# Hiroshiba/realtime-yukarin

Measured on NVIDIA H100. Metric: chunks_per_s_0.3s_24kHz_encode_stage1_stage2_vocode, higher is better.
Workload: dtype f64 (WORLD analysis / synthesis, SPTK), f16 operands / f32 accumulate: stage-2 k4 layers on wgmma, stage-1 k4 layers on mma.sync inside the one-launch cluster kernel; f32 CUDA cores (3x3 / k3 edge layers)

## Files before the change

### realtime_yukarin_b200/csrc/conv.h

```cpp
#pragma once
#include <cuda.h>

#include "common.cuh"

namespace ryk {

enum Act { ACT_NONE = 0, ACT_LEAKY = 1, ACT_RELU = 2 };
enum DType { DT_F32 = 0, DT_F16 = 1 };

constexpr int kMaxGroupVoices = 8;
constexpr int kMaxGroupBatch = 64;

struct LayerWeights {
  const float* w[kMaxGroupVoices];
  const float* scale[kMaxGroupVoices];
  const float* shift[kMaxGroupVoices];
  float host_scale[kMaxGroupVoices], host_shift[kMaxGroupVoices];
  uint8_t voice_of[kMaxGroupBatch];
};
__host__ __device__ inline int item_voice(const LayerWeights& wt, int b) { return b < kMaxGroupBatch ? wt.voice_of[b] : 0; }
struct TcWeightMaps { CUtensorMap m[kMaxGroupVoices]; };

struct ConvLayer {
  int transposed = 0;
  int B = 1, Hin = 1, Win = 1, Hout = 1, Wout = 1;
  int C0 = 0, C1 = 0, Cout = 0;
  int KH = 1, KW = 1, SH = 1, SW = 1, PH = 0, PW = 0;
  int act = ACT_NONE;
  int band_y0 = 0, band_y1 = 0;
  int skip_y0 = 0, skip_y1 = 0;
  int run_y0 = 0, run_y1 = 0;
  const void* in0 = nullptr; const void* in1 = nullptr; int in_dtype = DT_F32;
  void* out = nullptr; int out_dtype = DT_F32;
  int n_voices = 1;
  LayerWeights wt = {};
  bool host_scale_valid = false;
  const __half* w_tc[kMaxGroupVoices] = {};
  const __half* w_frag = nullptr;
  int ksplit = 1;
  int ksplit_tiles = 0;
  CUtensorMap tmA0, tmA1, tmO;
  TcWeightMaps tmB;
  int tile_w = 0, tile_h = 0;
  int block_n = 0;
  bool tc_ready = false;
};

inline int layer_class_rows(const ConvLayer& L) { return L.transposed ? L.Hin : L.Hout; }
inline int layer_band_end(const ConvLayer& L) { return L.band_y1 > 0 ? L.band_y1 : layer_class_rows(L); }
inline void layer_band_out_rows(const ConvLayer& L, int* r0, int* r1) {
  const int s = L.transposed ? L.SH : 1;
  *r0 = L.band_y0 * s;
  *r1 = layer_band_end(L) * s < L.Hout ? layer_band_end(L) * s : L.Hout;
}

int pack_weights_direct(const float* d_w_chainer, int transposed, int Cin, int Cout, int KH, int KW, float* d_out, cudaStream_t st);
int pack_weights_tc(const float* d_w_chainer, int transposed, int Cin, int Cout, int KH, int KW, int SH, int SW, __half* d_out, cudaStream_t st);

int conv_direct_run(const ConvLayer& L, cudaStream_t st);
bool conv_direct_band_supported(const ConvLayer& L);
bool conv_direct_cin1(const ConvLayer& L);
constexpr int kCin1Rows = 8;
bool conv_direct_per_item_weights(const ConvLayer& L);

bool tc_layer_eligible(const ConvLayer& L);
int tc_init();
int tc_layer_prepare(ConvLayer& L, int num_sms);
int tc_layer_weight_maps(ConvLayer& L);
int conv_tc_run(const ConvLayer& L, cudaStream_t st);
int tc_tile_rows(const ConvLayer& L);
int tc_tile_count(const ConvLayer& L);

int s1_pack_weights(const float* d_w_chainer, int transposed, int Cin, int Cout, __half* d_out, cudaStream_t st);
int s1_fused_init();
int s1_fused_cluster_size();

}
```

### realtime_yukarin_b200/csrc/conv_tc.cu

```cuda
#include <cuda.h>
#include <cudaTypedefs.h>

#include "conv.h"
#include "tc_ptx.cuh"

namespace ryk {

struct TcParams {
  int transposed, B, Hout, Wout, Cout;
  int Hc, Wc;
  int tile_w, tile_h, tiles_w, tiles_h;
  int th0;
  int skip_t0, skip_tn;
  int run_y0, run_y1;
  int chunks0, chunks1;
  int taps_w, ntaps;
  int sh, sw, ph, pw;
  int classes_w;
  int ksplit, chunks_per_split;
  int act;
  LayerWeights wt;
  __half* out;
};

template <int BLOCK_N>
__device__ __forceinline__ void wgmma_tile(float (&acc)[BLOCK_N / 2], uint64_t adesc, uint64_t bdesc) {
  if constexpr (BLOCK_N == 128) wgmma_m64n128(acc, adesc, bdesc);
  else wgmma_m64n64(acc, adesc, bdesc);
}

constexpr int kMaxSplits = 16;

__device__ __forceinline__ void add4(float4& a, const float4& b) { a.x += b.x; a.y += b.y; a.z += b.z; a.w += b.w; }

__device__ __forceinline__ float4 splitk_sum(const float4 (&v)[kMaxSplits], int ks) {
  float4 a = v[0];
  if (ks <= 4) {
#pragma unroll
    for (int s = 1; s < 4; ++s) if (s < ks) add4(a, v[s]);
    return a;
  }
#pragma unroll
  for (int g = 0; g < 8; ++g) {
    float4 part = make_float4(0.f, 0.f, 0.f, 0.f);
    if (g < ks) add4(part, v[g]);
    if (g + 8 < ks) add4(part, v[g + 8]);
    if (g == 0) a = part; else add4(a, part);
  }
  return a;
}

template <int BLOCK_N>
__device__ __forceinline__ uint32_t partial_offset(int row, int c) { return (uint32_t)(row * BLOCK_N * 4 + ((c ^ (row & 7)) << 4)); }

template <int BLOCK_N, int kStages, int kMinBlocks>
__global__ void __launch_bounds__(kTcThreads, kMinBlocks)
k_conv_tc(const __grid_constant__ CUtensorMap tmA0, const __grid_constant__ CUtensorMap tmA1,
          const __grid_constant__ TcWeightMaps tmB, const __grid_constant__ CUtensorMap tmO, const __grid_constant__ TcParams p) {
  static_assert(BLOCK_N == 64 || BLOCK_N == 128, "BLOCK_N");
  extern __shared__ __align__(1024) uint8_t smem_raw[];
  constexpr uint32_t kABytes = kBlockM * kBlockK * 2;
  constexpr uint32_t kBBytes = BLOCK_N * kBlockK * 2;
  static_assert((size_t)kBlockM * BLOCK_N * 4 <= (size_t)kStages * (kABytes + kBBytes), "epilogue staging must fit the stage buffers");
  uint8_t* smem = (uint8_t*)(((uintptr_t)smem_raw + 1023) & ~(uintptr_t)1023);
  uint8_t* smem_a = smem;
  uint8_t* smem_b = smem + kStages * kABytes;
  uint64_t* full_bar = (uint64_t*)(smem_b + kStages * kBBytes);
  uint64_t* empty_bar = full_bar + kStages;
  float* s_scale = (float*)(((uintptr_t)(empty_bar + kStages) + 15) & ~(uintptr_t)15);
  float* s_shift = s_scale + BLOCK_N;

  const int warp = threadIdx.x >> 5;
  pdl_trigger();

  int mt = blockIdx.x;
  const int tw = mt % p.tiles_w; mt /= p.tiles_w;
  int th = mt % p.tiles_h + p.th0; mt /= p.tiles_h;
  th += th >= p.skip_t0 ? p.skip_tn : 0;
  const int b = mt;
  const int n0 = blockIdx.y * BLOCK_N;
  const int cls = blockIdx.z / p.ksplit, split = blockIdx.z % p.ksplit;
  const int py = cls / p.classes_w, px = cls % p.classes_w;
  const int oy0 = th * p.tile_h, ox0 = tw * p.tile_w;
  const int chunks_per_tap = p.chunks0 + p.chunks1;
  const int total_chunks = p.ntaps * chunks_per_tap;
  const int kc_begin = split * p.chunks_per_split;
  const int kc_end = min(total_chunks, kc_begin + p.chunks_per_split);
  const int my_chunks = kc_end - kc_begin;
  const int voice = item_voice(p.wt, b);
  const CUtensorMap* tmBv = &tmB.m[voice];

  if (threadIdx.x == kTcConsumers) {
    asm volatile("prefetch.tensormap [%0];" ::"l"(&tmA0) : "memory");
    asm volatile("prefetch.tensormap [%0];" ::"l"(tmBv) : "memory");
    if (p.chunks1 > 0) asm volatile("prefetch.tensormap [%0];" ::"l"(&tmA1) : "memory");
    if (p.ksplit == 1) asm volatile("prefetch.tensormap [%0];" ::"l"(&tmO) : "memory");
    for (int i = 0; i < kStages; ++i) { mbar_init(&full_bar[i], 1); mbar_init(&empty_bar[i], kTcConsumers / 32); }
    asm volatile("fence.mbarrier_init.release.cluster;" ::: "memory");
  }
  if (threadIdx.x < kTcConsumers) {
    const float* scale = p.wt.scale[voice]; const float* shift = p.wt.shift[voice];
    for (int i = threadIdx.x; i < BLOCK_N; i += kTcConsumers) { s_scale[i] = __ldg(scale + n0 + i); s_shift[i] = __ldg(shift + n0 + i); }
  }
  __syncthreads();
  pdl_wait();

  if (warp == kTcConsumers / 32) {
    for (int i = 0; i < my_chunks; ++i) {
      const int s = i % kStages;
      const uint32_t ph = (i / kStages) & 1;
      mbar_wait(&empty_bar[s], ph ^ 1);
      const int kc = kc_begin + i;
      const int tap = kc / chunks_per_tap;
      const int cc = kc - tap * chunks_per_tap;
      const int ty = tap / p.taps_w, tx = tap - ty * p.taps_w;
      int ix, iy;
      if (!p.transposed) {
        ix = ox0 * p.sw + tx - p.pw; iy = oy0 * p.sh + ty - p.ph;
        if (iy >= p.run_y0 && iy + p.sh * (p.tile_h - 1) < p.run_y1) iy = p.run_y0;
      }
      else {
        ix = p.sw == 2 ? ox0 + tx - 1 + px : ox0;
        iy = p.sh == 2 ? oy0 + ty - 1 + py : oy0;
      }
      if (elect_one()) {
        mbar_expect_tx(&full_bar[s], kABytes + kBBytes);
        if (cc < p.chunks0) tma_load_4d(smem_a + s * kABytes, &tmA0, &full_bar[s], cc * kBlockK, ix, iy, b);
        else tma_load_4d(smem_a + s * kABytes, &tmA1, &full_bar[s], (cc - p.chunks0) * kBlockK, ix, iy, b);
        tma_load_2d(smem_b + s * kBBytes, tmBv, &full_bar[s], kc * kBlockK, cls * p.Cout + n0);
      }
    }
    if (p.ksplit > 1) { cluster_sync_all(); cluster_sync_all(); }
  } else if (warp < kTcConsumers / 32) {
    const int g = threadIdx.x >> 7, wl = warp & 3, lane = threadIdx.x & 31;
    float acc[BLOCK_N / 2];
#pragma unroll
    for (int i = 0; i < BLOCK_N / 2; ++i) acc[i] = 0.f;
    wgmma_fence_acc(acc);
    for (int i = 0; i < my_chunks; ++i) {
      const int s = i % kStages;
      mbar_wait(&full_bar[s], (i / kStages) & 1);
      const uint64_t adesc = make_sw128_desc(smem_u32(smem_a + s * kABytes + g * (64 * 128)));
      const uint64_t bdesc = make_sw128_desc(smem_u32(smem_b + s * kBBytes));
      wgmma_fence();
#pragma unroll
      for (int k = 0; k < kBlockK / kMmaK; ++k) wgmma_tile<BLOCK_N>(acc, adesc + (uint64_t)(k * 2), bdesc + (uint64_t)(k * 2));
      wgmma_commit();
      wgmma_wait<1>();
      wgmma_fence_acc(acc);
      if (i > 0) {
        __syncwarp();
        if (lane == 0) mbar_arrive(&empty_bar[(i - 1) % kStages]);
      }
    }
    wgmma_wait<0>();
    wgmma_fence_acc(acc);
    asm volatile("bar.sync 1, %0;" ::"n"(kTcConsumers) : "memory");
    const int rbase = g * 64 + wl * 16 + (lane >> 2);
    const int cq = 2 * (lane & 3);
    if (p.ksplit > 1) {
#pragma unroll
      for (int i = 0; i < BLOCK_N / 2; i += 2) {
        const int row = rbase + 8 * ((i >> 1) & 1);
        const int col = 8 * (i >> 2) + cq;
        *reinterpret_cast<float2*>(smem + partial_offset<BLOCK_N>(row, col >> 2) + (col & 3) * 4) = make_float2(acc[i], acc[i + 1]);
      }
      cluster_sync_all();
      const int vw = min(p.tile_w, p.Wc - ox0), vh = min(p.tile_h, p.Hc - oy0);
      constexpr int kChunks = BLOCK_N / 4;
      const int total = vw * vh * kChunks;
      const int j1 = (int)((long long)total * (split + 1) / p.ksplit);
      const uint32_t partial = smem_u32(smem);
      for (int j = (int)((long long)total * split / p.ksplit) + threadIdx.x; j < j1; j += kTcConsumers) {
        const int q = j / kChunks, c = j - q * kChunks;
        const int y = q / vw, x = q - y * vw;
        const uint32_t off = partial + partial_offset<BLOCK_N>(y * p.tile_w + x, c);
        float4 v[kMaxSplits];
#pragma unroll
        for (int s = 0; s < kMaxSplits; ++s)
          if (s < p.ksplit) v[s] = ld_cluster_f4(cluster_map(off, s));
        const float4 a = splitk_sum(v, p.ksplit);
        const int n = 4 * c;
        float o[4] = {fmaf(a.x, s_scale[n], s_shift[n]), fmaf(a.y, s_scale[n + 1], s_shift[n + 1]),
                      fmaf(a.z, s_scale[n + 2], s_shift[n + 2]), fmaf(a.w, s_scale[n + 3], s_shift[n + 3])};
#pragma unroll
        for (int k = 0; k < 4; ++k) {
          if (p.act == ACT_LEAKY) o[k] = o[k] > 0.f ? o[k] : 0.2f * o[k]; else if (p.act == ACT_RELU) o[k] = fmaxf(o[k], 0.f);
        }
        const int ys = p.transposed ? (oy0 + y) * p.sh + py : oy0 + y;
        const int xs = p.transposed ? (ox0 + x) * p.sw + px : ox0 + x;
        __half2 h0 = __floats2half2_rn(o[0], o[1]), h1 = __floats2half2_rn(o[2], o[3]);
        *reinterpret_cast<uint2*>(p.out + (((size_t)b * p.Hout + ys) * p.Wout + xs) * p.Cout + n0 + n) =
            make_uint2(*reinterpret_cast<uint32_t*>(&h0), *reinterpret_cast<uint32_t*>(&h1));
      }
      cluster_sync_all();
      return;
    }
#pragma unroll
    for (int i = 0; i < BLOCK_N / 2; i += 2) {
      const int row = rbase + 8 * ((i >> 1) & 1);
      const int col = 8 * (i >> 2) + cq;
      float v0 = fmaf(acc[i], s_scale[col], s_shift[col]);
      float v1 = fmaf(acc[i + 1], s_scale[col + 1], s_shift[col + 1]);
      if (p.act == ACT_LEAKY) { v0 = v0 > 0.f ? v0 : 0.2f * v0; v1 = v1 > 0.f ? v1 : 0.2f * v1; }
      else if (p.act == ACT_RELU) { v0 = fmaxf(v0, 0.f); v1 = fmaxf(v1, 0.f); }
      uint8_t* blk = smem + (col >> 6) * (kBlockM * 128) + row * 128;
      *reinterpret_cast<__half2*>(blk + ((((col & 63) >> 3) ^ (row & 7)) << 4) + (col & 7) * 2) = __floats2half2_rn(v0, v1);
    }
    if (my_chunks > 0) {
      asm volatile("fence.proxy.async.shared::cta;" ::: "memory");
      asm volatile("bar.sync 1, %0;" ::"n"(kTcConsumers) : "memory");
      if (threadIdx.x == 0) {
        const int xs = p.transposed ? ox0 * p.sw + px : ox0;
        const int ys = p.transposed ? oy0 * p.sh + py : oy0;
#pragma unroll
        for (int jb = 0; jb < BLOCK_N / 64; ++jb)
          asm volatile("cp.async.bulk.tensor.4d.global.shared::cta.bulk_group [%0, {%2, %3, %4, %5}], [%1];"
                       ::"l"(&tmO), "r"(smem_u32(smem + jb * (kBlockM * 128))), "r"(n0 + jb * 64), "r"(xs), "r"(ys), "r"(b) : "memory");
        asm volatile("cp.async.bulk.commit_group;" ::: "memory");
        asm volatile("cp.async.bulk.wait_group.read 0;" ::: "memory");
      }
    }
  }
}

static PFN_cuTensorMapEncodeTiled_v12000 g_encode = nullptr;
static int g_clusters[kMaxSplits + 1] = {};

template <int BN, int ST> static constexpr size_t tc_smem_bytes() {
  return (size_t)ST * (kBlockM * kBlockK * 2 + BN * kBlockK * 2) + 2 * ST * 8 + 16 + 1024 + 2 * BN * 4 + 32;
}
#define RYK_TC_N128 k_conv_tc<128, 3, 2>
#define RYK_TC_N64 k_conv_tc<64, 4, 2>

int tc_init() {
  if (!g_encode) {
    void* fn = nullptr;
    cudaDriverEntryPointQueryResult qres;
    RYK_CUDA(cudaGetDriverEntryPoint("cuTensorMapEncodeTiled", &fn, cudaEnableDefault, &qres));
    RYK_CHECK(qres == cudaDriverEntryPointSuccess && fn != nullptr, "cuTensorMapEncodeTiled not available from the driver");
    g_encode = (PFN_cuTensorMapEncodeTiled_v12000)fn;
  }
  RYK_CUDA(cudaFuncSetAttribute(RYK_TC_N128, cudaFuncAttributeMaxDynamicSharedMemorySize, (int)tc_smem_bytes<128, 3>()));
  RYK_CUDA(cudaFuncSetAttribute(RYK_TC_N64, cudaFuncAttributeMaxDynamicSharedMemorySize, (int)tc_smem_bytes<64, 4>()));
  RYK_CUDA(cudaFuncSetAttribute(RYK_TC_N128, cudaFuncAttributeNonPortableClusterSizeAllowed, 1));
  RYK_CUDA(cudaFuncSetAttribute(RYK_TC_N64, cudaFuncAttributeNonPortableClusterSizeAllowed, 1));
  if (g_clusters[1] == 0) {
    auto active = [](auto kernel, size_t smem, int ks) {
      cudaLaunchConfig_t cfg = {};
      cfg.gridDim = dim3(1, 1, ks); cfg.blockDim = dim3(kTcThreads); cfg.dynamicSmemBytes = smem;
      cudaLaunchAttribute at[1];
      at[0].id = cudaLaunchAttributeClusterDimension; at[0].val.clusterDim.x = 1; at[0].val.clusterDim.y = 1; at[0].val.clusterDim.z = ks;
      cfg.attrs = at; cfg.numAttrs = 1;
      int n = 0;
      if (cudaOccupancyMaxActiveClusters(&n, kernel, &cfg) != cudaSuccess) { cudaGetLastError(); n = 0; }
      return n;
    };
    for (int ks = 1; ks <= kMaxSplits; ++ks)
      g_clusters[ks] = std::min(active(RYK_TC_N128, tc_smem_bytes<128, 3>(), ks), active(RYK_TC_N64, tc_smem_bytes<64, 4>(), ks));
    RYK_CHECK(g_clusters[1] > 0, "the tensor-core convolution kernel does not fit an SM");
  }
  return 0;
}


bool tc_layer_eligible(const ConvLayer& L) {
  const bool k2d = L.KH == 4 && L.KW == 4 && L.SH == 2 && L.SW == 2 && L.PH == 1 && L.PW == 1;
  const bool k1d = L.KH == 1 && L.KW == 4 && L.SH == 1 && L.SW == 2 && L.PH == 0 && L.PW == 1;
  if (!k2d && !k1d) return false;
  if (L.C0 % kBlockK != 0 || L.C1 % kBlockK != 0 || L.C0 == 0) return false;
  if (L.Cout % 64 != 0) return false;
  if (L.in_dtype != DT_F16 || L.out_dtype != DT_F16) return false;
  return true;
}

static int pow2_floor(int v) { int p = 1; while (p * 2 <= v) p *= 2; return p; }

static int make_act_map(CUtensorMap* m, const void* ptr, int C, int W, int H, int B, int box_w, int box_h, int stride_w, int stride_h) {
  cuuint64_t dims[4] = {(cuuint64_t)C, (cuuint64_t)W, (cuuint64_t)H, (cuuint64_t)B};
  cuuint64_t strides[3] = {(cuuint64_t)C * 2, (cuuint64_t)W * C * 2, (cuuint64_t)H * W * C * 2};
  cuuint32_t box[4] = {(cuuint32_t)kBlockK, (cuuint32_t)(box_w * stride_w), (cuuint32_t)(box_h * stride_h), 1};
  cuuint32_t estr[4] = {1, (cuuint32_t)stride_w, (cuuint32_t)stride_h, 1};
  CUresult r = g_encode(m, CU_TENSOR_MAP_DATA_TYPE_FLOAT16, 4, const_cast<void*>(ptr), dims, strides, box, estr,
                        CU_TENSOR_MAP_INTERLEAVE_NONE, CU_TENSOR_MAP_SWIZZLE_128B, CU_TENSOR_MAP_L2_PROMOTION_L2_256B,
                        CU_TENSOR_MAP_FLOAT_OOB_FILL_NONE);
  if (r != CUDA_SUCCESS) { set_error("cuTensorMapEncodeTiled(activation) failed: " + std::to_string((int)r)); return -1; }
  return 0;
}

static int make_weight_map(CUtensorMap* m, const void* ptr, size_t K, size_t rows, int block_n) {
  cuuint64_t dims[2] = {(cuuint64_t)K, (cuuint64_t)rows};
  cuuint64_t strides[1] = {(cuuint64_t)K * 2};
  cuuint32_t box[2] = {(cuuint32_t)kBlockK, (cuuint32_t)block_n};
  cuuint32_t estr[2] = {1, 1};
  CUresult r = g_encode(m, CU_TENSOR_MAP_DATA_TYPE_FLOAT16, 2, const_cast<void*>(ptr), dims, strides, box, estr,
                        CU_TENSOR_MAP_INTERLEAVE_NONE, CU_TENSOR_MAP_SWIZZLE_128B, CU_TENSOR_MAP_L2_PROMOTION_L2_256B,
                        CU_TENSOR_MAP_FLOAT_OOB_FILL_NONE);
  if (r != CUDA_SUCCESS) { set_error("cuTensorMapEncodeTiled(weights) failed: " + std::to_string((int)r)); return -1; }
  return 0;
}

static void tc_tile_shape(const ConvLayer& L, int* tile_w, int* tile_h) {
  const int Wc = L.transposed ? L.Win : L.Wout;
  *tile_w = pow2_floor(Wc < kBlockM ? Wc : kBlockM);
  *tile_h = kBlockM / *tile_w;
}

int tc_tile_rows(const ConvLayer& L) { int tw, th; tc_tile_shape(L, &tw, &th); return th; }

int tc_tile_count(const ConvLayer& L) {
  int tw, th;
  tc_tile_shape(L, &tw, &th);
  const int Wc = L.transposed ? L.Win : L.Wout;
  const int band_tiles_h = (layer_band_end(L) - L.band_y0 + th - 1) / th;
  const int bn = L.Cout >= 128 ? 128 : 64;
  const int classes = L.transposed ? L.SH * L.SW : 1;
  return L.B * ((Wc + tw - 1) / tw) * band_tiles_h * (L.Cout / bn) * classes;
}

static void tc_geometry(const ConvLayer& L, int num_sms, int* tile_w, int* tile_h, int* block_n, int* ksplit) {
  int tw, th;
  tc_tile_shape(L, &tw, &th);
  int bn = L.Cout >= 128 ? 128 : 64;
  int tiles = L.ksplit_tiles > 0 ? L.ksplit_tiles : tc_tile_count(L);
  int ntaps = L.transposed ? (L.KH / L.SH) * (L.KW / L.SW) : L.KH * L.KW;
  int total_chunks = ntaps * (L.C0 + L.C1) / kBlockK;
  int ks = 1;
  int slots = num_sms * 2;
  if (tiles < slots) {
    constexpr int kMinChunks = 8;
    ks = slots / tiles;
    if (ks > total_chunks / kMinChunks) ks = total_chunks / kMinChunks;
    if (ks > kMaxSplits) ks = kMaxSplits;
    if (ks < 1) ks = 1;
    while (ks > 1 && tiles > g_clusters[ks]) --ks;
    int cps = (total_chunks + ks - 1) / ks;
    ks = (total_chunks + cps - 1) / cps;
  }
  *tile_w = tw; *tile_h = th; *block_n = bn; *ksplit = ks;
}

int tc_layer_weight_maps(ConvLayer& L) {
  RYK_CHECK(L.n_voices >= 1 && L.n_voices <= kMaxGroupVoices, "a layer holds 1..8 voices");
  const int classes = L.transposed ? L.SH * L.SW : 1;
  const int ntaps = L.transposed ? (L.KH / L.SH) * (L.KW / L.SW) : L.KH * L.KW;
  const size_t K = (size_t)ntaps * (L.C0 + L.C1), rows = (size_t)classes * L.Cout;
  for (int v = 0; v < L.n_voices; ++v) {
    RYK_CHECK(L.w_tc[v] != nullptr, "tensor-core layer without packed weights for one of its voices");
    if (make_weight_map(&L.tmB.m[v], L.w_tc[v], K, rows, L.block_n)) return -1;
  }
  for (int v = L.n_voices; v < kMaxGroupVoices; ++v) L.tmB.m[v] = L.tmB.m[0];
  return 0;
}

int tc_layer_prepare(ConvLayer& L, int num_sms) {
  RYK_CHECK(g_encode != nullptr, "tc_init() was not called");
  RYK_CHECK(tc_layer_eligible(L), "layer is not eligible for the tensor-core path");
  tc_geometry(L, num_sms, &L.tile_w, &L.tile_h, &L.block_n, &L.ksplit);
  int stw = L.transposed ? 1 : L.SW, sth = L.transposed ? 1 : L.SH;
  if (make_act_map(&L.tmA0, L.in0, L.C0, L.Win, L.Hin, L.B, L.tile_w, L.tile_h, stw, sth)) return -1;
  if (L.C1 > 0) { if (make_act_map(&L.tmA1, L.in1, L.C1, L.Win, L.Hin, L.B, L.tile_w, L.tile_h, stw, sth)) return -1; }
  else L.tmA1 = L.tmA0;
  if (tc_layer_weight_maps(L)) return -1;
  if (make_act_map(&L.tmO, L.out, L.Cout, L.Wout, L.Hout, L.B, L.tile_w, L.tile_h, L.transposed ? L.SW : 1, L.transposed ? L.SH : 1)) return -1;
  RYK_CHECK(L.band_y0 >= 0 && L.band_y0 % L.tile_h == 0 && L.band_y0 < layer_band_end(L) && layer_band_end(L) <= layer_class_rows(L) &&
            (layer_band_end(L) % L.tile_h == 0 || layer_band_end(L) == layer_class_rows(L)), "row band is not a range of whole tile rows");
  RYK_CHECK(L.skip_y1 == 0 || (!L.transposed && L.skip_y0 % L.tile_h == 0 && L.skip_y1 % L.tile_h == 0 && L.band_y0 <= L.skip_y0 &&
                               L.skip_y0 < L.skip_y1 && L.skip_y1 <= layer_band_end(L)),
            "skipped rows are not a range of whole tile rows inside the band of a convolution");
  L.tc_ready = true;
  return 0;
}

template <typename... KArgs, typename... Args>
static cudaError_t launch_pdl(void (*kernel)(KArgs...), dim3 grid, dim3 block, size_t smem, cudaStream_t st, int cluster_z, Args&&... args) {
  cudaLaunchConfig_t cfg = {};
  cfg.gridDim = grid; cfg.blockDim = block; cfg.dynamicSmemBytes = smem; cfg.stream = st;
  cudaLaunchAttribute attr[2];
  attr[0].id = cudaLaunchAttributeProgrammaticStreamSerialization; attr[0].val.programmaticStreamSerializationAllowed = 1;
  attr[1].id = cudaLaunchAttributeClusterDimension; attr[1].val.clusterDim.x = 1; attr[1].val.clusterDim.y = 1; attr[1].val.clusterDim.z = cluster_z;
  cfg.attrs = attr; cfg.numAttrs = cluster_z > 1 ? 2 : 1;
  return cudaLaunchKernelEx(&cfg, kernel, static_cast<KArgs>(args)...);
}

int conv_tc_run(const ConvLayer& L, cudaStream_t st) {
  RYK_CHECK(L.tc_ready, "tc layer not prepared");
  TcParams p;
  p.transposed = L.transposed; p.B = L.B; p.Hout = L.Hout; p.Wout = L.Wout; p.Cout = L.Cout;
  p.Hc = L.transposed ? L.Hin : L.Hout; p.Wc = L.transposed ? L.Win : L.Wout;
  p.tile_w = L.tile_w; p.tile_h = L.tile_h;
  p.skip_t0 = L.skip_y0 / L.tile_h; p.skip_tn = (L.skip_y1 - L.skip_y0) / L.tile_h;
  p.tiles_w = (p.Wc + L.tile_w - 1) / L.tile_w; p.tiles_h = (layer_band_end(L) - L.band_y0 + L.tile_h - 1) / L.tile_h - p.skip_tn;
  p.th0 = L.band_y0 / L.tile_h;
  p.run_y0 = L.run_y0; p.run_y1 = L.run_y1;
  p.chunks0 = L.C0 / kBlockK; p.chunks1 = L.C1 / kBlockK;
  p.taps_w = L.transposed ? L.KW / L.SW : L.KW;
  p.ntaps = L.transposed ? (L.KH / L.SH) * (L.KW / L.SW) : L.KH * L.KW;
  p.sh = L.SH; p.sw = L.SW; p.ph = L.PH; p.pw = L.PW;
  p.classes_w = L.transposed ? L.SW : 1;
  const int classes = L.transposed ? L.SH * L.SW : 1;
  p.ksplit = L.ksplit;
  int total_chunks = p.ntaps * (p.chunks0 + p.chunks1);
  p.chunks_per_split = (total_chunks + L.ksplit - 1) / L.ksplit;
  p.act = L.act; p.wt = L.wt;
  p.out = (__half*)L.out;
  dim3 grid(L.B * p.tiles_w * p.tiles_h, L.Cout / L.block_n, classes * L.ksplit);
  if (L.block_n == 128) RYK_CUDA(launch_pdl(RYK_TC_N128, grid, dim3(kTcThreads), tc_smem_bytes<128, 3>(), st, L.ksplit, L.tmA0, L.tmA1, L.tmB, L.tmO, p));
  else RYK_CUDA(launch_pdl(RYK_TC_N64, grid, dim3(kTcThreads), tc_smem_bytes<64, 4>(), st, L.ksplit, L.tmA0, L.tmA1, L.tmB, L.tmO, p));
  RYK_CUDA(cudaGetLastError());
  return 0;
}

}
```

### realtime_yukarin_b200/csrc/tc_ptx.cuh

```cuda
#pragma once
#include <cuda.h>
#include <stdint.h>

namespace ryk {

constexpr int kBlockM = 128;
constexpr int kBlockK = 64;
constexpr int kMmaK = 16;
constexpr int kTcConsumers = 256;
constexpr int kTcThreads = kTcConsumers + 32;

__device__ __forceinline__ uint32_t smem_u32(const void* p) { return (uint32_t)__cvta_generic_to_shared(p); }

__device__ __forceinline__ void pdl_trigger() { asm volatile("griddepcontrol.launch_dependents;" ::: "memory"); }
__device__ __forceinline__ void pdl_wait() { asm volatile("griddepcontrol.wait;" ::: "memory"); }

__device__ __forceinline__ bool elect_one() {
  uint32_t pred;
  asm volatile("{\n\t.reg .pred p;\n\telect.sync _|p, 0xffffffff;\n\tselp.u32 %0, 1, 0, p;\n\t}" : "=r"(pred));
  return pred != 0;
}

__device__ __forceinline__ void mbar_init(uint64_t* bar, uint32_t count) {
  asm volatile("mbarrier.init.shared::cta.b64 [%0], %1;" ::"r"(smem_u32(bar)), "r"(count));
}
__device__ __forceinline__ void mbar_expect_tx(uint64_t* bar, uint32_t bytes) {
  asm volatile("mbarrier.arrive.expect_tx.shared::cta.b64 _, [%0], %1;" ::"r"(smem_u32(bar)), "r"(bytes) : "memory");
}
__device__ __forceinline__ void mbar_arrive(uint64_t* bar) {
  asm volatile("mbarrier.arrive.shared::cta.b64 _, [%0];" ::"r"(smem_u32(bar)) : "memory");
}
__device__ __forceinline__ void mbar_wait(uint64_t* bar, uint32_t parity) {
  asm volatile(
      "{\n\t"
      ".reg .pred p;\n\t"
      "WAIT_LOOP:\n\t"
      "mbarrier.try_wait.parity.shared::cta.b64 p, [%0], %1;\n\t"
      "@p bra WAIT_DONE;\n\t"
      "bra WAIT_LOOP;\n\t"
      "WAIT_DONE:\n\t"
      "}" ::"r"(smem_u32(bar)), "r"(parity) : "memory");
}
__device__ __forceinline__ void tma_load_4d(void* dst, const CUtensorMap* map, uint64_t* bar, int c0, int c1, int c2, int c3) {
  asm volatile(
      "cp.async.bulk.tensor.4d.shared::cluster.global.mbarrier::complete_tx::bytes [%0], [%1, {%3, %4, %5, %6}], [%2];"
      ::"r"(smem_u32(dst)), "l"(map), "r"(smem_u32(bar)), "r"(c0), "r"(c1), "r"(c2), "r"(c3) : "memory");
}
__device__ __forceinline__ void tma_load_2d(void* dst, const CUtensorMap* map, uint64_t* bar, int c0, int c1) {
  asm volatile(
      "cp.async.bulk.tensor.2d.shared::cluster.global.mbarrier::complete_tx::bytes [%0], [%1, {%3, %4}], [%2];"
      ::"r"(smem_u32(dst)), "l"(map), "r"(smem_u32(bar)), "r"(c0), "r"(c1) : "memory");
}
__device__ __forceinline__ void wgmma_fence() { asm volatile("wgmma.fence.sync.aligned;" ::: "memory"); }
__device__ __forceinline__ void wgmma_commit() { asm volatile("wgmma.commit_group.sync.aligned;" ::: "memory"); }
template <int N> __device__ __forceinline__ void wgmma_wait() { asm volatile("wgmma.wait_group.sync.aligned %0;" ::"n"(N) : "memory"); }
template <int R> __device__ __forceinline__ void wgmma_fence_acc(float (&d)[R]) {
#pragma unroll
  for (int i = 0; i < R; ++i) asm volatile("" : "+f"(d[i])::"memory");
}
__device__ __forceinline__ void wgmma_m64n64(float (&d)[32], uint64_t adesc, uint64_t bdesc) {
  asm volatile(
      "{\n\t.reg .pred p;\n\tsetp.ne.b32 p, %34, 0;\n\t"
      "wgmma.mma_async.sync.aligned.m64n64k16.f32.f16.f16 "
      "{%0, %1, %2, %3, %4, %5, %6, %7, %8, %9, %10, %11, %12, %13, %14, %15, %16, %17, %18, %19, %20, %21, %22, %23, %24, %25, %26, %27, %28, %29, %30, %31}, "
      "%32, %33, p, 1, 1, 0, 0;\n\t}"
      : "+f"(d[0]), "+f"(d[1]), "+f"(d[2]), "+f"(d[3]), "+f"(d[4]), "+f"(d[5]), "+f"(d[6]), "+f"(d[7]), "+f"(d[8]), "+f"(d[9]), "+f"(d[10]), "+f"(d[11]), "+f"(d[12]), "+f"(d[13]), "+f"(d[14]), "+f"(d[15]), "+f"(d[16]), "+f"(d[17]), "+f"(d[18]), "+f"(d[19]), "+f"(d[20]), "+f"(d[21]), "+f"(d[22]), "+f"(d[23]), "+f"(d[24]), "+f"(d[25]), "+f"(d[26]), "+f"(d[27]), "+f"(d[28]), "+f"(d[29]), "+f"(d[30]), "+f"(d[31])
      : "l"(adesc), "l"(bdesc), "r"(1));
}
__device__ __forceinline__ void wgmma_m64n128(float (&d)[64], uint64_t adesc, uint64_t bdesc) {
  asm volatile(
      "{\n\t.reg .pred p;\n\tsetp.ne.b32 p, %66, 0;\n\t"
      "wgmma.mma_async.sync.aligned.m64n128k16.f32.f16.f16 "
      "{%0, %1, %2, %3, %4, %5, %6, %7, %8, %9, %10, %11, %12, %13, %14, %15, %16, %17, %18, %19, %20, %21, %22, %23, %24, %25, %26, %27, %28, %29, %30, %31, %32, %33, %34, %35, %36, %37, %38, %39, %40, %41, %42, %43, %44, %45, %46, %47, %48, %49, %50, %51, %52, %53, %54, %55, %56, %57, %58, %59, %60, %61, %62, %63}, "
      "%64, %65, p, 1, 1, 0, 0;\n\t}"
      : "+f"(d[0]), "+f"(d[1]), "+f"(d[2]), "+f"(d[3]), "+f"(d[4]), "+f"(d[5]), "+f"(d[6]), "+f"(d[7]), "+f"(d[8]), "+f"(d[9]), "+f"(d[10]), "+f"(d[11]), "+f"(d[12]), "+f"(d[13]), "+f"(d[14]), "+f"(d[15]), "+f"(d[16]), "+f"(d[17]), "+f"(d[18]), "+f"(d[19]), "+f"(d[20]), "+f"(d[21]), "+f"(d[22]), "+f"(d[23]), "+f"(d[24]), "+f"(d[25]), "+f"(d[26]), "+f"(d[27]), "+f"(d[28]), "+f"(d[29]), "+f"(d[30]), "+f"(d[31]), "+f"(d[32]), "+f"(d[33]), "+f"(d[34]), "+f"(d[35]), "+f"(d[36]), "+f"(d[37]), "+f"(d[38]), "+f"(d[39]), "+f"(d[40]), "+f"(d[41]), "+f"(d[42]), "+f"(d[43]), "+f"(d[44]), "+f"(d[45]), "+f"(d[46]), "+f"(d[47]), "+f"(d[48]), "+f"(d[49]), "+f"(d[50]), "+f"(d[51]), "+f"(d[52]), "+f"(d[53]), "+f"(d[54]), "+f"(d[55]), "+f"(d[56]), "+f"(d[57]), "+f"(d[58]), "+f"(d[59]), "+f"(d[60]), "+f"(d[61]), "+f"(d[62]), "+f"(d[63])
      : "l"(adesc), "l"(bdesc), "r"(1));
}
__device__ __forceinline__ uint32_t cluster_rank() { uint32_t r; asm volatile("mov.u32 %0, %%cluster_ctarank;" : "=r"(r)); return r; }
__device__ __forceinline__ void cluster_sync_all() {
  asm volatile("barrier.cluster.arrive.release.aligned;\n\tbarrier.cluster.wait.acquire.aligned;" ::: "memory");
}
__device__ __forceinline__ uint32_t cluster_map(uint32_t a, uint32_t rank) {
  uint32_t r;
  asm volatile("mapa.shared::cluster.u32 %0, %1, %2;" : "=r"(r) : "r"(a), "r"(rank));
  return r;
}
__device__ __forceinline__ float4 ld_cluster_f4(uint32_t a) {
  float4 v;
  asm volatile("ld.shared::cluster.v4.f32 {%0, %1, %2, %3}, [%4];" : "=f"(v.x), "=f"(v.y), "=f"(v.z), "=f"(v.w) : "r"(a) : "memory");
  return v;
}

__device__ __forceinline__ uint64_t make_sw128_desc(uint32_t smem_addr) {
  uint64_t d = 0;
  d |= (uint64_t)((smem_addr >> 4) & 0x3FFF);
  d |= (uint64_t)1 << 16;
  d |= (uint64_t)((1024u >> 4) & 0x3FFF) << 32;
  d |= (uint64_t)1 << 62;
  return d;
}


}
```

Measured before the change: 2628.

## Load a shared input patch once per tap pair for k4 tensor-core convs

Adds a patch mode to the wgmma convolution kernel for kernel-height-4 layers with wide tiles. Each pipeline stage now loads one (tile_w+1)-wide input patch via a strided 5D plane tensor map (or a widened 4D map for transposed layers) together with two weight blocks. The two horizontally adjacent taps then share that patch by offsetting the A descriptor by one row. This halves the number of pipeline steps and cuts redundant activation traffic through TMA, at the cost of larger stages, fewer pipeline stages, and more complex addressing.

Result: faster. 2674 (median of 6 runs) (+1.8%).

```diff
diff --git a/realtime_yukarin_b200/csrc/conv.h b/realtime_yukarin_b200/csrc/conv.h
--- a/realtime_yukarin_b200/csrc/conv.h
+++ b/realtime_yukarin_b200/csrc/conv.h
@@ -43,6 +43,7 @@
   TcWeightMaps tmB;
   int tile_w = 0, tile_h = 0;
   int block_n = 0;
+  bool tc_patch = false;
   bool tc_ready = false;
 };
 
diff --git a/realtime_yukarin_b200/csrc/conv_tc.cu b/realtime_yukarin_b200/csrc/conv_tc.cu
--- a/realtime_yukarin_b200/csrc/conv_tc.cu
+++ b/realtime_yukarin_b200/csrc/conv_tc.cu
@@ -1,5 +1,7 @@
 #include <cuda.h>
 #include <cudaTypedefs.h>
+
+#include <algorithm>
 
 #include "conv.h"
 #include "tc_ptx.cuh"
@@ -17,7 +19,7 @@
   int taps_w, ntaps;
   int sh, sw, ph, pw;
   int classes_w;
-  int ksplit, chunks_per_split;
+  int ksplit, steps_per_split;
   int act;
   LayerWeights wt;
   __half* out;
@@ -53,19 +55,25 @@
 template <int BLOCK_N>
 __device__ __forceinline__ uint32_t partial_offset(int row, int c) { return (uint32_t)(row * BLOCK_N * 4 + ((c ^ (row & 7)) << 4)); }
 
-template <int BLOCK_N, int kStages, int kMinBlocks>
+constexpr uint32_t kPatchBytes = 17 * 1024;
+template <int BLOCK_N, bool kPatch> constexpr uint32_t tc_stage_bytes() {
+  return kPatch ? kPatchBytes + 2 * BLOCK_N * kBlockK * 2 : kBlockM * kBlockK * 2 + BLOCK_N * kBlockK * 2;
+}
+
+template <int BLOCK_N, int kStages, int kMinBlocks, bool kPatch>
 __global__ void __launch_bounds__(kTcThreads, kMinBlocks)
 k_conv_tc(const __grid_constant__ CUtensorMap tmA0, const __grid_constant__ CUtensorMap tmA1,
           const __grid_constant__ TcWeightMaps tmB, const __grid_constant__ CUtensorMap tmO, const __grid_constant__ TcParams p) {
   static_assert(BLOCK_N == 64 || BLOCK_N == 128, "BLOCK_N");
   extern __shared__ __align__(1024) uint8_t smem_raw[];
-  constexpr uint32_t kABytes = kBlockM * kBlockK * 2;
+  constexpr uint32_t kABytes = kPatch ? kPatchBytes : kBlockM * kBlockK * 2;
   constexpr uint32_t kBBytes = BLOCK_N * kBlockK * 2;
-  static_assert((size_t)kBlockM * BLOCK_N * 4 <= (size_t)kStages * (kABytes + kBBytes), "epilogue staging must fit the stage buffers");
+  constexpr uint32_t kStageBytes = tc_stage_bytes<BLOCK_N, kPatch>();
+  static_assert((size_t)kBlockM * BLOCK_N * 4 <= (size_t)kStages * kStageBytes, "epilogue staging must fit the stage buffers");
   uint8_t* smem = (uint8_t*)(((uintptr_t)smem_raw + 1023) & ~(uintptr_t)1023);
   uint8_t* smem_a = smem;
   uint8_t* smem_b = smem + kStages * kABytes;
-  uint64_t* full_bar = (uint64_t*)(smem_b + kStages * kBBytes);
+  uint64_t* full_bar = (uint64_t*)(smem + kStages * kStageBytes);
   uint64_t* empty_bar = full_bar + kStages;
   float* s_scale = (float*)(((uintptr_t)(empty_bar + kStages) + 15) & ~(uintptr_t)15);
   float* s_shift = s_scale + BLOCK_N;
@@ -83,10 +91,10 @@
   const int py = cls / p.classes_w, px = cls % p.classes_w;
   const int oy0 = th * p.tile_h, ox0 = tw * p.tile_w;
   const int chunks_per_tap = p.chunks0 + p.chunks1;
-  const int total_chunks = p.ntaps * chunks_per_tap;
-  const int kc_begin = split * p.chunks_per_split;
-  const int kc_end = min(total_chunks, kc_begin + p.chunks_per_split);
-  const int my_chunks = kc_end - kc_begin;
+  const int total_steps = p.ntaps * chunks_per_tap / (kPatch ? 2 : 1);
+  const int kc_begin = split * p.steps_per_split;
+  const int kc_end = min(total_steps, kc_begin + p.steps_per_split);
+  const int my_steps = kc_end - kc_begin;
   const int voice = item_voice(p.wt, b);
   const CUtensorMap* tmBv = &tmB.m[voice];
 
@@ -106,11 +114,34 @@
   pdl_wait();
 
   if (warp == kTcConsumers / 32) {
-    for (int i = 0; i < my_chunks; ++i) {
+    for (int i = 0; i < my_steps; ++i) {
       const int s = i % kStages;
       const uint32_t ph = (i / kStages) & 1;
       mbar_wait(&empty_bar[s], ph ^ 1);
       const int kc = kc_begin + i;
+      if constexpr (kPatch) {
+        const int planes = p.transposed ? 1 : 2;
+        const int q = kc % planes, tc = kc / planes;
+        const int ty = tc / chunks_per_tap, cc = tc - ty * chunks_per_tap;
+        const int tap0 = ty * p.taps_w + q;
+        if (elect_one()) {
+          uint8_t* stage = smem + s * kStageBytes;
+          mbar_expect_tx(&full_bar[s], p.tile_h * (p.tile_w + 1) * 128 + 2 * kBBytes);
+          const CUtensorMap* tmA = cc < p.chunks0 ? &tmA0 : &tmA1;
+          const int c0 = (cc < p.chunks0 ? cc : cc - p.chunks0) * kBlockK;
+          if (!p.transposed) {
+            const int ix = ox0 * 2 + q - p.pw;
+            int iy = oy0 * p.sh + ty - p.ph;
+            if (iy >= p.run_y0 && iy + p.sh * (p.tile_h - 1) < p.run_y1) iy = p.run_y0;
+            tma_load_5d(stage, tmA, &full_bar[s], c0, ix & 1, ix >> 1, iy, b);
+          } else {
+            tma_load_4d(stage, tmA, &full_bar[s], c0, ox0 - 1 + px, oy0 + ty - 1 + py, b);
+          }
+          tma_load_2d(stage + kABytes, tmBv, &full_bar[s], (tap0 * chunks_per_tap + cc) * kBlockK, cls * p.Cout + n0);
+          tma_load_2d(stage + kABytes + kBBytes, tmBv, &full_bar[s], ((tap0 + planes) * chunks_per_tap + cc) * kBlockK, cls * p.Cout + n0);
+        }
+        continue;
+      }
       const int tap = kc / chunks_per_tap;
       const int cc = kc - tap * chunks_per_tap;
       const int ty = tap / p.taps_w, tx = tap - ty * p.taps_w;
@@ -137,14 +168,27 @@
 #pragma unroll
     for (int i = 0; i < BLOCK_N / 2; ++i) acc[i] = 0.f;
     wgmma_fence_acc(acc);
-    for (int i = 0; i < my_chunks; ++i) {
+    const int prow = kPatch ? (64 * g / p.tile_w) * (p.tile_w + 1) + (64 * g) % p.tile_w : 0;
+    for (int i = 0; i < my_steps; ++i) {
       const int s = i % kStages;
       mbar_wait(&full_bar[s], (i / kStages) & 1);
-      const uint64_t adesc = make_sw128_desc(smem_u32(smem_a + s * kABytes + g * (64 * 128)));
-      const uint64_t bdesc = make_sw128_desc(smem_u32(smem_b + s * kBBytes));
-      wgmma_fence();
-#pragma unroll
-      for (int k = 0; k < kBlockK / kMmaK; ++k) wgmma_tile<BLOCK_N>(acc, adesc + (uint64_t)(k * 2), bdesc + (uint64_t)(k * 2));
+      if constexpr (kPatch) {
+        const uint32_t a = smem_u32(smem + s * kStageBytes) + prow * 128;
+        const uint64_t adesc0 = make_sw128_desc(a), adesc1 = make_sw128_desc(a + 128);
+        const uint64_t bdesc0 = make_sw128_desc(smem_u32(smem + s * kStageBytes + kABytes));
+        const uint64_t bdesc1 = make_sw128_desc(smem_u32(smem + s * kStageBytes + kABytes + kBBytes));
+        wgmma_fence();
+#pragma unroll
+        for (int k = 0; k < kBlockK / kMmaK; ++k) wgmma_tile<BLOCK_N>(acc, adesc0 + (uint64_t)(k * 2), bdesc0 + (uint64_t)(k * 2));
+#pragma unroll
+        for (int k = 0; k < kBlockK / kMmaK; ++k) wgmma_tile<BLOCK_N>(acc, adesc1 + (uint64_t)(k * 2), bdesc1 + (uint64_t)(k * 2));
+      } else {
+        const uint64_t adesc = make_sw128_desc(smem_u32(smem_a + s * kABytes + g * (64 * 128)));
+        const uint64_t bdesc = make_sw128_desc(smem_u32(smem_b + s * kBBytes));
+        wgmma_fence();
+#pragma unroll
+        for (int k = 0; k < kBlockK / kMmaK; ++k) wgmma_tile<BLOCK_N>(acc, adesc + (uint64_t)(k * 2), bdesc + (uint64_t)(k * 2));
+      }
       wgmma_commit();
       wgmma_wait<1>();
       wgmma_fence_acc(acc);
@@ -207,7 +251,7 @@
       uint8_t* blk = smem + (col >> 6) * (kBlockM * 128) + row * 128;
       *reinterpret_cast<__half2*>(blk + ((((col & 63) >> 3) ^ (row & 7)) << 4) + (col & 7) * 2) = __floats2half2_rn(v0, v1);
     }
-    if (my_chunks > 0) {
+    if (my_steps > 0) {
       asm volatile("fence.proxy.async.shared::cta;" ::: "memory");
       asm volatile("bar.sync 1, %0;" ::"n"(kTcConsumers) : "memory");
       if (threadIdx.x == 0) {
@@ -227,11 +271,15 @@
 static PFN_cuTensorMapEncodeTiled_v12000 g_encode = nullptr;
 static int g_clusters[kMaxSplits + 1] = {};
 
-template <int BN, int ST> static constexpr size_t tc_smem_bytes() {
-  return (size_t)ST * (kBlockM * kBlockK * 2 + BN * kBlockK * 2) + 2 * ST * 8 + 16 + 1024 + 2 * BN * 4 + 32;
-}
-#define RYK_TC_N128 k_conv_tc<128, 3, 2>
-#define RYK_TC_N64 k_conv_tc<64, 4, 2>
+template <int BN, int ST, bool PATCH> static constexpr size_t tc_smem_bytes() {
+  return (size_t)ST * tc_stage_bytes<BN, PATCH>() + 2 * ST * 8 + 16 + 1024 + 2 * BN * 4 + 32;
+}
+#define RYK_TC_N128 k_conv_tc<128, 3, 2, false>
+#define RYK_TC_N64 k_conv_tc<64, 4, 2, false>
+#define RYK_TC_P128 k_conv_tc<128, 2, 2, true>
+#define RYK_TC_P64 k_conv_tc<64, 3, 2, true>
+static constexpr size_t kSmemN128 = tc_smem_bytes<128, 3, false>(), kSmemN64 = tc_smem_bytes<64, 4, false>();
+static constexpr size_t kSmemP128 = tc_smem_bytes<128, 2, true>(), kSmemP64 = tc_smem_bytes<64, 3, true>();
 
 int tc_init() {
   if (!g_encode) {
@@ -241,10 +289,12 @@
     RYK_CHECK(qres == cudaDriverEntryPointSuccess && fn != nullptr, "cuTensorMapEncodeTiled not available from the driver");
     g_encode = (PFN_cuTensorMapEncodeTiled_v12000)fn;
   }
-  RYK_CUDA(cudaFuncSetAttribute(RYK_TC_N128, cudaFuncAttributeMaxDynamicSharedMemorySize, (int)tc_smem_bytes<128, 3>()));
-  RYK_CUDA(cudaFuncSetAttribute(RYK_TC_N64, cudaFuncAttributeMaxDynamicSharedMemorySize, (int)tc_smem_bytes<64, 4>()));
-  RYK_CUDA(cudaFuncSetAttribute(RYK_TC_N128, cudaFuncAttributeNonPortableClusterSizeAllowed, 1));
-  RYK_CUDA(cudaFuncSetAttribute(RYK_TC_N64, cudaFuncAttributeNonPortableClusterSizeAllowed, 1));
+  auto attrs = [](auto kernel, size_t smem) -> int {
+    RYK_CUDA(cudaFuncSetAttribute(kernel, cudaFuncAttributeMaxDynamicSharedMemorySize, (int)smem));
+    RYK_CUDA(cudaFuncSetAttribute(kernel, cudaFuncAttributeNonPortableClusterSizeAllowed, 1));
+    return 0;
+  };
+  if (attrs(RYK_TC_N128, kSmemN128) || attrs(RYK_TC_N64, kSmemN64) || attrs(RYK_TC_P128, kSmemP128) || attrs(RYK_TC_P64, kSmemP64)) return -1;
   if (g_clusters[1] == 0) {
     auto active = [](auto kernel, size_t smem, int ks) {
       cudaLaunchConfig_t cfg = {};
@@ -257,7 +307,8 @@
       return n;
     };
     for (int ks = 1; ks <= kMaxSplits; ++ks)
-      g_clusters[ks] = std::min(active(RYK_TC_N128, tc_smem_bytes<128, 3>(), ks), active(RYK_TC_N64, tc_smem_bytes<64, 4>(), ks));
+      g_clusters[ks] = std::min({active(RYK_TC_N128, kSmemN128, ks), active(RYK_TC_N64, kSmemN64, ks), active(RYK_TC_P128, kSmemP128, ks),
+                                 active(RYK_TC_P64, kSmemP64, ks)});
     RYK_CHECK(g_clusters[1] > 0, "the tensor-core convolution kernel does not fit an SM");
   }
   return 0;
@@ -288,6 +339,18 @@
   return 0;
 }
 
+static int make_plane_map(CUtensorMap* m, const void* ptr, int C, int W, int H, int B, int tile_w, int tile_h, int stride_h) {
+  cuuint64_t dims[5] = {(cuuint64_t)C, 2, (cuuint64_t)W / 2, (cuuint64_t)H, (cuuint64_t)B};
+  cuuint64_t strides[4] = {(cuuint64_t)C * 2, (cuuint64_t)C * 4, (cuuint64_t)W * C * 2, (cuuint64_t)H * W * C * 2};
+  cuuint32_t box[5] = {(cuuint32_t)kBlockK, 1, (cuuint32_t)(tile_w + 1), (cuuint32_t)(tile_h * stride_h), 1};
+  cuuint32_t estr[5] = {1, 1, 1, (cuuint32_t)stride_h, 1};
+  CUresult r = g_encode(m, CU_TENSOR_MAP_DATA_TYPE_FLOAT16, 5, const_cast<void*>(ptr), dims, strides, box, estr,
+                        CU_TENSOR_MAP_INTERLEAVE_NONE, CU_TENSOR_MAP_SWIZZLE_128B, CU_TENSOR_MAP_L2_PROMOTION_L2_256B,
+                        CU_TENSOR_MAP_FLOAT_OOB_FILL_NONE);
+  if (r != CUDA_SUCCESS) { set_error("cuTensorMapEncodeTiled(plane) failed: " + std::to_string((int)r)); return -1; }
+  return 0;
+}
+
 static int make_weight_map(CUtensorMap* m, const void* ptr, size_t K, size_t rows, int block_n) {
   cuuint64_t dims[2] = {(cuuint64_t)K, (cuuint64_t)rows};
   cuuint64_t strides[1] = {(cuuint64_t)K * 2};
@@ -306,6 +369,10 @@
   *tile_h = kBlockM / *tile_w;
 }
 
+static bool tc_patch_path(const ConvLayer& L, int tile_w) {
+  return L.KH == 4 && tile_w >= 64 && (L.transposed || L.Win % 2 == 0);
+}
+
 int tc_tile_rows(const ConvLayer& L) { int tw, th; tc_tile_shape(L, &tw, &th); return th; }
 
 int tc_tile_count(const ConvLayer& L) {
@@ -325,6 +392,7 @@
   int tiles = L.ksplit_tiles > 0 ? L.ksplit_tiles : tc_tile_count(L);
   int ntaps = L.transposed ? (L.KH / L.SH) * (L.KW / L.SW) : L.KH * L.KW;
   int total_chunks = ntaps * (L.C0 + L.C1) / kBlockK;
+  int total_steps = tc_patch_path(L, tw) ? total_chunks / 2 : total_chunks;
   int ks = 1;
   int slots = num_sms * 2;
   if (tiles < slots) {
@@ -334,8 +402,8 @@
     if (ks > kMaxSplits) ks = kMaxSplits;
     if (ks < 1) ks = 1;
     while (ks > 1 && tiles > g_clusters[ks]) --ks;
-    int cps = (total_chunks + ks - 1) / ks;
-    ks = (total_chunks + cps - 1) / cps;
+    int sps = (total_steps + ks - 1) / ks;
+    ks = (total_steps + sps - 1) / sps;
   }
   *tile_w = tw; *tile_h = th; *block_n = bn; *ksplit = ks;
 }
@@ -357,9 +425,14 @@
   RYK_CHECK(g_encode != nullptr, "tc_init() was not called");
   RYK_CHECK(tc_layer_eligible(L), "layer is not eligible for the tensor-core path");
   tc_geometry(L, num_sms, &L.tile_w, &L.tile_h, &L.block_n, &L.ksplit);
-  int stw = L.transposed ? 1 : L.SW, sth = L.transposed ? 1 : L.SH;
-  if (make_act_map(&L.tmA0, L.in0, L.C0, L.Win, L.Hin, L.B, L.tile_w, L.tile_h, stw, sth)) return -1;
-  if (L.C1 > 0) { if (make_act_map(&L.tmA1, L.in1, L.C1, L.Win, L.Hin, L.B, L.tile_w, L.tile_h, stw, sth)) return -1; }
+  L.tc_patch = tc_patch_path(L, L.tile_w);
+  auto act_map = [&](CUtensorMap* m, const void* ptr, int C) {
+    if (L.tc_patch && !L.transposed) return make_plane_map(m, ptr, C, L.Win, L.Hin, L.B, L.tile_w, L.tile_h, L.SH);
+    if (L.tc_patch) return make_act_map(m, ptr, C, L.Win, L.Hin, L.B, L.tile_w + 1, L.tile_h, 1, 1);
+    return make_act_map(m, ptr, C, L.Win, L.Hin, L.B, L.tile_w, L.tile_h, L.transposed ? 1 : L.SW, L.transposed ? 1 : L.SH);
+  };
+  if (act_map(&L.tmA0, L.in0, L.C0)) return -1;
+  if (L.C1 > 0) { if (act_map(&L.tmA1, L.in1, L.C1)) return -1; }
   else L.tmA1 = L.tmA0;
   if (tc_layer_weight_maps(L)) return -1;
   if (make_act_map(&L.tmO, L.out, L.Cout, L.Wout, L.Hout, L.B, L.tile_w, L.tile_h, L.transposed ? L.SW : 1, L.transposed ? L.SH : 1)) return -1;
@@ -400,13 +473,16 @@
   p.classes_w = L.transposed ? L.SW : 1;
   const int classes = L.transposed ? L.SH * L.SW : 1;
   p.ksplit = L.ksplit;
-  int total_chunks = p.ntaps * (p.chunks0 + p.chunks1);
-  p.chunks_per_split = (total_chunks + L.ksplit - 1) / L.ksplit;
+  const int total_steps = p.ntaps * (p.chunks0 + p.chunks1) / (L.tc_patch ? 2 : 1);
+  p.steps_per_split = (total_steps + L.ksplit - 1) / L.ksplit;
   p.act = L.act; p.wt = L.wt;
   p.out = (__half*)L.out;
   dim3 grid(L.B * p.tiles_w * p.tiles_h, L.Cout / L.block_n, classes * L.ksplit);
-  if (L.block_n == 128) RYK_CUDA(launch_pdl(RYK_TC_N128, grid, dim3(kTcThreads), tc_smem_bytes<128, 3>(), st, L.ksplit, L.tmA0, L.tmA1, L.tmB, L.tmO, p));
-  else RYK_CUDA(launch_pdl(RYK_TC_N64, grid, dim3(kTcThreads), tc_smem_bytes<64, 4>(), st, L.ksplit, L.tmA0, L.tmA1, L.tmB, L.tmO, p));
+  const bool n128 = L.block_n == 128;
+  if (L.tc_patch && n128) RYK_CUDA(launch_pdl(RYK_TC_P128, grid, dim3(kTcThreads), kSmemP128, st, L.ksplit, L.tmA0, L.tmA1, L.tmB, L.tmO, p));
+  else if (L.tc_patch) RYK_CUDA(launch_pdl(RYK_TC_P64, grid, dim3(kTcThreads), kSmemP64, st, L.ksplit, L.tmA0, L.tmA1, L.tmB, L.tmO, p));
+  else if (n128) RYK_CUDA(launch_pdl(RYK_TC_N128, grid, dim3(kTcThreads), kSmemN128, st, L.ksplit, L.tmA0, L.tmA1, L.tmB, L.tmO, p));
+  else RYK_CUDA(launch_pdl(RYK_TC_N64, grid, dim3(kTcThreads), kSmemN64, st, L.ksplit, L.tmA0, L.tmA1, L.tmB, L.tmO, p));
   RYK_CUDA(cudaGetLastError());
   return 0;
 }
diff --git a/realtime_yukarin_b200/csrc/tc_ptx.cuh b/realtime_yukarin_b200/csrc/tc_ptx.cuh
--- a/realtime_yukarin_b200/csrc/tc_ptx.cuh
+++ b/realtime_yukarin_b200/csrc/tc_ptx.cuh
@@ -45,6 +45,11 @@
   asm volatile(
       "cp.async.bulk.tensor.4d.shared::cluster.global.mbarrier::complete_tx::bytes [%0], [%1, {%3, %4, %5, %6}], [%2];"
       ::"r"(smem_u32(dst)), "l"(map), "r"(smem_u32(bar)), "r"(c0), "r"(c1), "r"(c2), "r"(c3) : "memory");
+}
+__device__ __forceinline__ void tma_load_5d(void* dst, const CUtensorMap* map, uint64_t* bar, int c0, int c1, int c2, int c3, int c4) {
+  asm volatile(
+      "cp.async.bulk.tensor.5d.shared::cluster.global.mbarrier::complete_tx::bytes [%0], [%1, {%3, %4, %5, %6, %7}], [%2];"
+      ::"r"(smem_u32(dst)), "l"(map), "r"(smem_u32(bar)), "r"(c0), "r"(c1), "r"(c2), "r"(c3), "r"(c4) : "memory");
 }
 __device__ __forceinline__ void tma_load_2d(void* dst, const CUtensorMap* map, uint64_t* bar, int c0, int c1) {
   asm volatile(
```
